# numz/ComfyUI-SeedVR2_VideoUpscaler

Hardware: NVIDIA H100
Metric: upscaled frames/sec SeedVR2-3B 720p->4K (higher is better)
Workload: dtype bf16

## Files before the change

comfyui-seedvr2_videoupscaler_b200/csrc/gemm.cu:

```cuda
#include <cuda.h>
#include <cuda_runtime.h>
#include <cuda_bf16.h>
#include <stdint.h>
#include <stdio.h>
#include <stdlib.h>

#include <type_traits>

#include "ptx.cuh"
#include "svr2_internal.h"

namespace svr2 {

constexpr int BLOCK_M = 128;
constexpr int BLOCK_K = 64;
constexpr int WGMMA_K = 16;

struct GemmParams {
  int M, N, K;
  int num_m_tiles, num_n_tiles, num_k_blocks;
  int band_h;
  int group_n;
  int a_mode;
  int tiles_w, tiles_h;
// ... 20 lines not shown
  const __nv_bfloat16* residual;
  void* out;
  float4* stat_partial;
  int stat_slots;
  const float* rowscale;
  float2* stat2;
  int ld_stat;
  const int* run_if;
  void* out2;
  void* out3;
  const int32_t* tok_dst;
  const int32_t* tok_rope;
  const float* rope_cos;
  const float* rope_sin;
  const float* qk_weight;
  float qk_eps;
  int qkv_inner;
};

enum : int {
  EPI_BIAS = 1,
  EPI_GATE = 2,
  EPI_RESIDUAL = 4,
  EPI_SWIGLU = 8,
  EPI_GELU = 16,
  EPI_F32 = 32,
  EPI_SHUFFLE = 64,
  EPI_SILU = 128,
  EPI_ROWSTAT = 256,
  EPI_PEXP = 512,
  EPI_ROWSCALE = 1024,
};

template <int BLOCK_N, bool EPI_WG>
struct SmemLayout {
  static constexpr int kABytes = BLOCK_M * BLOCK_K * 2;
  static constexpr int kBBytes = BLOCK_N * BLOCK_K * 2;
  static constexpr int kStageBytes = kABytes + kBBytes;
  static constexpr int kTileCols = BLOCK_N < 32 ? 32 : BLOCK_N;
  static constexpr int kStagingBytes = EPI_WG ? BLOCK_M * kTileCols * 2 : 8 * 4096;
  static constexpr int kBudget = 232448 - kStagingBytes - 256 - 1024;
  static constexpr int kStages = kBudget / kStageBytes > 8 ? 8 : kBudget / kStageBytes;
  static constexpr int kStagingOffset = kStages * kStageBytes;
  static constexpr int kBarOffset = kStagingOffset + kStagingBytes;
  static constexpr int kTotal = kBarOffset + 256 + 1024;
};

template <bool SWAP>
struct SlabLayout : SmemLayout<256, true> {
  using Base = SmemLayout<256, true>;
  static constexpr int kWBytes = (SWAP ? BLOCK_M : 256) * BLOCK_K * 2;
  static constexpr int kSBytes = (SWAP ? 32 * 10 : 16 * 10) * BLOCK_K * 2;
  static constexpr int kSStages = SWAP ? 2 : 3;
  static constexpr int kWStages = (Base::kBudget - kSStages * kSBytes) / kWBytes;
  static constexpr int kStages = kWStages + kSStages;
  static constexpr int kSlabOffset = kWStages * kWBytes;
  static constexpr int kStagingOffset = kSlabOffset + kSStages * kSBytes;
  static constexpr int kBarOffset = kStagingOffset + Base::kStagingBytes;
  static constexpr int kTotal = kBarOffset + 256 + 1024;
  static_assert(kWStages >= 3 && kSBytes % 1024 == 0 && kTotal <= 232448, "slab rings do not fit");
};

__device__ __forceinline__ void acc_ld32(const float* acc, uint32_t idx, uint32_t (&v)[32]) {
  const float4* s = reinterpret_cast<const float4*>(acc + idx);
#pragma unroll
  for (int i = 0; i < 8; ++i) {
    const float4 t = s[i];
    v[4 * i] = __float_as_uint(t.x); v[4 * i + 1] = __float_as_uint(t.y);
    v[4 * i + 2] = __float_as_uint(t.z); v[4 * i + 3] = __float_as_uint(t.w);
  }
}

__device__ __forceinline__ void stat_acc(float4& a, const uint4& d) {
// ... 22 lines not shown
  const int r = m_blk - band * full;
  const int rows_left = p.tiles_h - band * p.band_h;
  const int rows = rows_left < p.band_h ? rows_left : p.band_h;
  const int per = rows * p.tiles_w;
  t_o = r / per;
  const int rr = r - t_o * per;
  const int trow = rr / p.tiles_w;
  th = band * p.band_h + trow;
  tw = rr - trow * p.tiles_w;
}

__device__ __forceinline__ int conv_k_blocks(const GemmParams& p, int m_blk) {
  if (p.fold_t == 0) return p.num_k_blocks;
  int t_o, th, tw;
  conv_tile(p, m_blk, t_o, th, tw);
  return t_o < p.fold_t ? p.num_k_blocks - (p.taps_t - 1 - t_o) * p.taps_h * p.taps_w * p.cin_blocks : p.num_k_blocks;
}

__device__ __forceinline__ void tile_coords(int tile, int num_m, int num_n, int g, int& m, int& n) {
  const int per_group = g * num_m;
  const int ng = tile / per_group;
  const int r = tile - ng * per_group;
  const int n0 = ng * g;
  const int gsz = (num_n - n0) < g ? (num_n - n0) : g;
  m = r / gsz;
  n = n0 + (r - m * gsz);
}

enum : int { KIND_BF16 = 0, KIND_SWIGLU = 1, KIND_F32 = 2, KIND_ROWSTAT = 3, KIND_PEXP = 4,
             KIND_QKV21 = 5, KIND_QKV10 = 6,
             KIND_BF16_RS = 7,
             KIND_PEXP_STAT = 8 };

template <int KIND> constexpr bool kEpiWG = KIND == KIND_BF16;
constexpr int kNumThreads = 384;
constexpr int kEpiWarps = 2;

__device__ __forceinline__ int swap_tile_swz(int pix) { return ((pix & 1) << 2) | ((pix >> 1) & 3); }

struct RowDest {
  long long off;
  int valid;
  int dup;
};

template <int BLOCK_N>
__device__ __forceinline__ RowDest row_dest(const GemmParams& p, int epi, int m_blk, int n_blk, int row, int n_cols) {
  RowDest d;
  d.dup = 0;
  if (epi & EPI_SHUFFLE) {
    const int m = m_blk * BLOCK_M + row;
    d.valid = m < p.M;
    const int hw = p.shuf_H * p.shuf_W;
    const int f = m / hw, rr = m - f * hw, h = rr / p.shuf_W, w = rr - h * p.shuf_W;
    const int grp = (n_blk * BLOCK_N) / p.shuf_c;
    const int z = grp % p.shuf_z, y = (grp / p.shuf_z) & 1, x = grp / (p.shuf_z * 2);
    int t_out = f * p.shuf_z + z;
    if (p.shuf_drop) {
      if (f == 0 && z == 1) d.valid = 0;
      if (f > 0) t_out -= 1;
    }
    const int Wo = p.shuf_W * 2;
    const long long pix = (long long)(2 * h + x) * Wo + (2 * w + y);
    d.off = (long long)(t_out + p.out_t_pad) * p.out_frame_stride + pix * p.ldc + ((n_blk * BLOCK_N) % p.shuf_c);
    d.dup = (p.out_dup_head && t_out == 0 && d.valid) ? 1 : 0;
  } else if (p.a_mode == 0) {
    const int m = m_blk * BLOCK_M + row;
    d.valid = m < p.M;
    d.off = (long long)m * p.ldc + (long long)n_blk * n_cols;
  } else {
    int t_o, th, tw;
    conv_tile(p, m_blk, t_o, th, tw);
    const int rh = row / p.bw;
    const int h = th * p.bh + rh;
    const int w = tw * p.bw + (row - rh * p.bw);
    d.valid = (h < p.H_out) && (w < p.W_out);
    d.off = (long long)(t_o + p.out_t_pad) * p.out_frame_stride + ((long long)h * p.W_out + w) * p.ldc +
            (long long)n_blk * BLOCK_N;
    d.dup = (p.out_dup_head && t_o == 0 && d.valid) ? 1 : 0;
  }
  return d;
}

template <int BLOCK_N, int KIND, bool SWAP = false, int EPI_CT = -1, bool SLAB = false>
__global__ void __launch_bounds__(kNumThreads, 1)
gemm_wgmma_kernel(const __grid_constant__ CUtensorMap tmap_a, const __grid_constant__ CUtensorMap tmap_b,
                  const __grid_constant__ CUtensorMap tmap_a2, const GemmParams p) {
  if (p.run_if != nullptr && *p.run_if == 0) return;
  constexpr bool EPI_WG = kEpiWG<KIND>;
  static_assert(EPI_WG || (!SWAP && EPI_CT < 0), "swap-AB and compile-time epilogues are KIND_BF16 only");
  static_assert(!SLAB || (KIND == KIND_BF16 && BLOCK_N == 256), "the slab mainloop is KIND_BF16 with 256-column tiles");
  using S = SlabLayout<SWAP>;
  using L = std::conditional_t<SLAB, S, SmemLayout<BLOCK_N, EPI_WG>>;
  constexpr int kStages = L::kStages;
  constexpr int ACC_STRIDE = BLOCK_N < 32 ? 32 : BLOCK_N;
  constexpr int ACC_LD = ACC_STRIDE + 4;
  static_assert(EPI_WG || BLOCK_M * ACC_LD * 4 <= L::kStagingOffset, "the accumulator tile overlays the operand ring");
  extern __shared__ uint8_t smem_raw[];
  uint8_t* smem = reinterpret_cast<uint8_t*>((reinterpret_cast<uintptr_t>(smem_raw) + 1023) & ~uintptr_t(1023));
  uint64_t* full_bar = reinterpret_cast<uint64_t*>(smem + L::kBarOffset);
  uint64_t* empty_bar = full_bar + kStages;
  uint64_t* acc_free = empty_bar + kStages;
  uint64_t* tile_full = acc_free + 1;
  uint64_t* tile_empty = acc_free + 2;
  const float* acc_s = reinterpret_cast<const float*>(smem);
  uint8_t* tile_s = smem + L::kStagingOffset;

  const int warp = threadIdx.x >> 5;
  const int lane = threadIdx.x & 31;

  if (warp == 0 && lane == 0) {
    tma_prefetch_desc(&tmap_a);
    tma_prefetch_desc(&tmap_b);
    if (p.extra_blocks) tma_prefetch_desc(&tmap_a2);
  }
  if (warp == 1 && lane == 0) {
    for (int i = 0; i < kStages; ++i) {
      mbar_init(&full_bar[i], 1);
      mbar_init(&empty_bar[i], 2);
    }
    if constexpr (EPI_WG) {
      mbar_init(tile_full, 256);
      mbar_init(tile_empty, 32 * kEpiWarps);
    } else {
      mbar_init(acc_free, 256);
    }
    fence_barrier_init();
  }
  __syncthreads();

  const int num_n_tiles = p.num_n_tiles;
  const int num_m_tiles = p.num_m_tiles;
  const int num_tiles = num_m_tiles * num_n_tiles;
  const int tile0 = (int)blockIdx.x;
  const int tile_step = (int)gridDim.x;

  if (warp == 0 || warp == 3) {
    if constexpr (SLAB) {
      if (lane == 0) {
        const bool wgt = warp == 0;
        const int n_st = wgt ? S::kWStages : S::kSStages;
        const int bar0 = wgt ? 0 : S::kWStages;
        const int st_bytes = wgt ? S::kWBytes : S::kSBytes;
        uint8_t* const ring = smem + (wgt ? 0 : S::kSlabOffset);
        int stage = 0;
        uint32_t phase = 0;
        auto acquire = [&](uint32_t bytes, uint64_t*& fb) -> uint8_t* {
          mbar_wait(&empty_bar[bar0 + stage], phase ^ 1);
          fb = &full_bar[bar0 + stage];
          mbar_expect_tx(fb, bytes);
          uint8_t* s = ring + stage * st_bytes;
          if (++stage == n_st) { stage = 0; phase ^= 1; }
          return s;
        };
        const int bw = p.bw, bh = p.bh, taps_t = p.taps_t, cin_blocks = p.cin_blocks, cin = p.cin;
        const uint32_t slab_bytes = bw * (bh + 2) * BLOCK_K * 2, box_bytes = bw * bh * BLOCK_K * 2;
        for (int tile = tile0; tile < num_tiles; tile += tile_step) {
          int m_blk, n_blk, t_o, th, tw;
          tile_coords(tile, num_m_tiles, num_n_tiles, p.group_n, m_blk, n_blk);
          conv_tile(p, m_blk, t_o, th, tw);
          const int h0 = th * bh, w0 = tw * bw;
          int n0 = n_blk * (SWAP ? BLOCK_M : BLOCK_N);
          int taps = taps_t, kcol = 0;
          if (t_o < p.fold_t) {
            taps = t_o + 1;
            kcol = t_o == 0 ? 2 * 9 * cin : 0;
            n0 += p.fold_n;
          }
          uint64_t* fb;
          for (int kt_ = 0; kt_ < taps; ++kt_) {
// ... 2 lines not shown
              for (int cb = 0; cb < cin_blocks; ++cb) {
                if (wgt) {
                  for (int kh_ = 0; kh_ < 3; ++kh_) {
                    uint8_t* s = acquire(S::kWBytes, fb);
                    tma_load_2d(s, &tmap_b, fb, kcol + ((kt_ * 3 + kh_) * 3 + kw_) * cin + cb * BLOCK_K, n0);
                  }
                } else {
                  uint8_t* s = acquire(slab_bytes, fb);
                  tma_load_4d(s, &tmap_a, fb, cb * BLOCK_K, w0 + kw_ - p.pad_w, h0 - p.pad_h, t_in);
                }
              }
            }
          }
          kcol += taps * 9 * cin;
          for (int cb = 0; cb < p.extra_blocks; ++cb) {
            if (wgt) {
              uint8_t* s = acquire(S::kWBytes, fb);
              tma_load_2d(s, &tmap_b, fb, kcol + cb * BLOCK_K, n0);
            } else {
              uint8_t* s = acquire(box_bytes, fb);
              tma_load_4d(s, &tmap_a2, fb, cb * BLOCK_K, w0, h0, t_o);
            }
          }
        }
      }
    } else if (lane == 0) {
      int stage = 0;
      uint32_t phase = 0;
      uint32_t g = (warp == 0) ? 0u : 1u;
      uint32_t it = 0;
      const int a_mode = p.a_mode;
      const int nkb = p.num_k_blocks;
      auto acquire = [&](uint8_t*& sa, uint64_t*& fb) -> bool {
        const bool mine = (g++ & 1u) == 0u;
        if (mine) {
          mbar_wait(&empty_bar[stage], phase ^ 1);
          sa = smem + stage * L::kStageBytes;
          fb = &full_bar[stage];
          mbar_expect_tx(fb, L::kStageBytes);
        }
        return mine;
      };
      auto advance = [&]() {
        if (++stage == kStages) { stage = 0; phase ^= 1; }
      };
      auto tile_start = [&]() {
        if (!EPI_WG && it > 0) mbar_wait(acc_free, (it - 1) & 1u);
        ++it;
      };
      if (a_mode == 0) {
        for (int tile = tile0; tile < num_tiles; tile += tile_step) {
          int m_blk, n_blk;
          tile_coords(tile, num_m_tiles, num_n_tiles, p.group_n, m_blk, n_blk);
          tile_start();
          const int m0 = m_blk * BLOCK_M, n0 = n_blk * BLOCK_N;
          for (int kb = 0; kb < nkb; ++kb) {
            uint8_t* sa; uint64_t* fb;
            if (acquire(sa, fb)) {
              tma_load_2d(sa, &tmap_a, fb, kb * BLOCK_K, m0);
              tma_load_2d(sa + L::kABytes, &tmap_b, fb, kb * BLOCK_K, n0);
            }
            advance();
          }
        }
      } else {
        const int bw = p.bw, bh = p.bh, pad_h = p.pad_h, pad_w = p.pad_w, stride_t = p.stride_t;
        const int taps_t = p.taps_t, taps_h = p.taps_h, taps_w = p.taps_w, cin_blocks = p.cin_blocks, cin = p.cin;
// ... 147 lines not shown
#pragma unroll
          for (int i = 0; i < BLOCK_N / 2; i += 8) {
            const int pix = (i >> 3) * 16 + ((mj >> 1) << 3) + lr;
            stmatrix_x4_trans(tbase + pix * 256 + ((chunk ^ swap_tile_swz(pix)) << 4),
                              pack_bf16x2(d[i] + b0, d[i + 1] + b0), pack_bf16x2(d[i + 2] + b1, d[i + 3] + b1),
                              pack_bf16x2(d[i + 4] + b0, d[i + 5] + b0), pack_bf16x2(d[i + 6] + b1, d[i + 7] + b1));
          }
        } else {
          constexpr int ROW_B = L::kTileCols * 2;
          constexpr int SWZ = (L::kTileCols / 8 < 8 ? L::kTileCols / 8 : 8) - 1;
          const int row = r0 + ((mj & 1) << 3) + lr;
          const int cn0 = n_blk * BLOCK_N + 2 * (lane & 3);
#pragma unroll
          for (int i = 0; i < BLOCK_N / 2; i += 8) {
            float x[8];
#pragma unroll
            for (int e = 0; e < 8; ++e) x[e] = d[i + e];
            if (epi & EPI_BIAS) {
              const int cn = cn0 + (i >> 3) * 16;
              const uint32_t bl = cn < p.N ? __ldg(reinterpret_cast<const unsigned int*>(bias + cn)) : 0u;
              const uint32_t bh = cn + 8 < p.N ? __ldg(reinterpret_cast<const unsigned int*>(bias + cn + 8)) : 0u;
              x[0] += __uint_as_float(bl << 16); x[1] += __uint_as_float(bl & 0xffff0000u);
              x[2] += __uint_as_float(bl << 16); x[3] += __uint_as_float(bl & 0xffff0000u);
              x[4] += __uint_as_float(bh << 16); x[5] += __uint_as_float(bh & 0xffff0000u);
              x[6] += __uint_as_float(bh << 16); x[7] += __uint_as_float(bh & 0xffff0000u);
            }
            const int chunk = (i >> 3) * 2 + (mj >> 1);
            stmatrix_x4(tbase + row * ROW_B + ((chunk ^ (row & SWZ)) << 4), pack_bf16x2(x[0], x[1]),
                        pack_bf16x2(x[2], x[3]), pack_bf16x2(x[4], x[5]), pack_bf16x2(x[6], x[7]));
          }
        }
        mbar_arrive(tile_full);
      };
      for (int tile = tile0; tile < num_tiles; tile += tile_step, ++it) {
        int m_blk, n_blk;
        tile_coords(tile, num_m_tiles, num_n_tiles, p.group_n, m_blk, n_blk);
        auto store = [&](float (&d)[BLOCK_N / 2]) { store_tile(d, n_blk); };
        if constexpr (SLAB) mainloop_slab(conv_k_blocks(p, m_blk), store);
        else mainloop(conv_k_blocks(p, m_blk), store);
      }
    } else {
      auto acc_to_smem = [&](float (&d)[BLOCK_N / 2]) {
        named_bar_sync(1, 256);
        float* acc_w = reinterpret_cast<float*>(smem);
        const int r0 = wg * 64 + ((warp & 3) << 4) + (lane >> 2);
#pragma unroll
        for (int i = 0; i < BLOCK_N / 2; i += 4) {
          const int col = (i >> 2) * 8 + 2 * (lane & 3);
          *reinterpret_cast<float2*>(acc_w + r0 * ACC_LD + col) = make_float2(d[i], d[i + 1]);
          *reinterpret_cast<float2*>(acc_w + (r0 + 8) * ACC_LD + col) = make_float2(d[i + 2], d[i + 3]);
        }
        named_bar_sync(1, 256);
      };
      constexpr bool IS_BF16 = KIND == KIND_BF16_RS;
      constexpr bool IS_PEXP = KIND == KIND_PEXP || KIND == KIND_PEXP_STAT;
      constexpr int N_COLS = KIND == KIND_SWIGLU ? ACC_STRIDE / 2 : ACC_STRIDE;
      constexpr int COLS_W = N_COLS >= 64 ? N_COLS / 2 : N_COLS;
      constexpr int PH_COLS = KIND == KIND_F32 ? 32 : (COLS_W < 64 ? COLS_W : 64);
      constexpr int CPR = KIND == KIND_F32 ? PH_COLS / 4 : PH_COLS / 8;
      constexpr int ROWS_PER_IT = 32 / CPR;
      constexpr int N_IT = 32 / ROWS_PER_IT;
      constexpr int kBatch = N_IT < 4 ? N_IT : 4;
      const int q = warp & 3;
      const int half = (warp - 4) >> 2;
      const int row = q * 32 + lane;
      const bool active = (N_COLS >= 64) || (half == 0);
      const int col_lo = (N_COLS >= 64) ? half * COLS_W : 0;
      uint8_t* slab = smem + L::kStagingOffset + (warp - 4) * 4096;
      const int n_lim = KIND == KIND_SWIGLU ? p.N / 2 : p.N;
      const float* __restrict__ gate = p.gate;
      const __nv_bfloat16* __restrict__ resid = p.residual;
      for (int tile = tile0; tile < num_tiles; tile += tile_step) {
        int m_blk, n_blk;
        tile_coords(tile, num_m_tiles, num_n_tiles, p.group_n, m_blk, n_blk);
        if (it++ > 0) {
          fence_proxy_async_smem();
          mbar_arrive(acc_free);
        }
        mainloop(conv_k_blocks(p, m_blk), acc_to_smem);
        RowDest dst = row_dest<BLOCK_N>(p, epi, m_blk, n_blk, row, N_COLS);
        const int n_base = n_blk * (KIND == KIND_SWIGLU ? BLOCK_N / 2 : BLOCK_N);

        constexpr bool kWide = (IS_BF16 || IS_PEXP) && PH_COLS == 64;
        constexpr int N_PH = kWide ? COLS_W / 64 : 1;
        uint32_t bias_pk[N_PH];
        float2 gate2[N_PH];
        if constexpr (kWide && IS_BF16) {
#pragma unroll
          for (int ph = 0; ph < N_PH; ++ph) {
            const int cn = n_base + col_lo + ph * 64 + 2 * lane;
            const bool ok = cn < p.N;
            bias_pk[ph] = ((epi & EPI_BIAS) && ok) ? *reinterpret_cast<const uint32_t*>(bias + cn) : 0u;
            gate2[ph] = ((epi & EPI_GATE) && ok) ? *reinterpret_cast<const float2*>(gate + cn) : make_float2(0.f, 0.f);
          }
        }

        const uint32_t t_addr = row * ACC_LD;

        float row_lse = 0.f;
        float2 st_a = make_float2(0.f, 0.f), st_b = make_float2(0.f, 0.f);
        if constexpr (IS_PEXP) {
          const int m = m_blk * BLOCK_M + row;
          row_lse = (m < p.M) ? gate[m] : 0.f;
        }
        float row_scale = 1.f;
        if constexpr (KIND == KIND_BF16_RS) {
          const int m = m_blk * BLOCK_M + row;
          row_scale = (p.a_mode == 0 && m < p.M) ? p.rowscale[m] : 1.f;
        }
        if constexpr (KIND == KIND_QKV21 || KIND == KIND_QKV10) {
          static_assert(BLOCK_N == 256, "QKV epilogue needs 256-column tiles");
          constexpr int NF = KIND == KIND_QKV21 ? 21 : 10;
          const int tpw = p.qkv_inner / 256;
          const int which = n_blk / tpw;
          const int m = m_blk * BLOCK_M + row;
          const bool rvalid = (m < p.M);
          uint32_t pk[64];
#pragma unroll
          for (int c0 = 0; c0 < 128; c0 += 64) {
            uint32_t v0[32], v1[32];
            acc_ld32(acc_s, t_addr + col_lo + c0, v0);
            acc_ld32(acc_s, t_addr + col_lo + c0 + 32, v1);
#pragma unroll
            for (int i = 0; i < 16; ++i) {
              pk[c0 / 2 + i] = pack_bf16x2(__uint_as_float(v0[2 * i]), __uint_as_float(v0[2 * i + 1]));
              pk[c0 / 2 + 16 + i] = pack_bf16x2(__uint_as_float(v1[2 * i]), __uint_as_float(v1[2 * i + 1]));
            }
          }
          if (which < 2) {
            float ss = 0.f;
#pragma unroll
            for (int i = 0; i < 64; ++i) {
              const float lo = __uint_as_float(pk[i] << 16), hi = __uint_as_float(pk[i] & 0xffff0000u);
// ... 75 lines not shown
                float cm = -INFINITY;
#pragma unroll
                for (int j = 0; j < RS; ++j) {
                  const float t = (n0 + j < p.N) ? __uint_as_float(v[j]) * sc : -INFINITY;
                  v[j] = __float_as_uint(t);
                  cm = fmaxf(cm, t);
                }
                const float m_new = fmaxf(mx, cm);
                if (m_new > -INFINITY) {
                  float cs = 0.f;
#pragma unroll
                  for (int j = 0; j < RS; ++j) cs += exp2_approx(__uint_as_float(v[j]) - m_new);
                  sum = sum * exp2_approx(mx - m_new) + cs;
                  mx = m_new;
                }
              }
            }
          }
          const int m = m_blk * BLOCK_M + row;
          if (active && m < p.M) {
            const int slot = (N_COLS >= 64) ? n_blk * 2 + half : n_blk;
            reinterpret_cast<float2*>(p.out)[(long long)m * p.ldc + slot] = make_float2(mx, sum);
          }
        } else if (active) {
#pragma unroll 1
          for (int ph0 = col_lo; ph0 < col_lo + COLS_W; ph0 += PH_COLS) {
            if constexpr (kWide) {
              uint32_t v0[32], v1[32];
              acc_ld32(acc_s, t_addr + ph0, v0);
              acc_ld32(acc_s, t_addr + ph0 + 32, v1);
              const int phi = (ph0 - col_lo) / 64;
              uint32_t pk[32];
              const float sc = p.out_scale;
              constexpr bool want_stats = KIND == KIND_PEXP_STAT;
              const bool stats_full = n_base + ph0 + 64 <= p.N;
              const bool plain = !(epi & (EPI_GELU | EPI_SILU | EPI_GATE));
              auto elements = [&](auto ragged) {
#pragma unroll
              for (int i = 0; i < 32; ++i) {
                float a = __uint_as_float(i < 16 ? v0[2 * (i & 15)] : v1[2 * (i & 15)]);
                float b = __uint_as_float(i < 16 ? v0[2 * (i & 15) + 1] : v1[2 * (i & 15) + 1]);
                if constexpr (IS_PEXP) {
                  const bool kPoly = (KIND == KIND_PEXP_STAT) && ((i % 5 == 1) || (i % 5 == 3));
                  const float xa = fmaf(a, sc, -row_lse), xb = fmaf(b, sc, -row_lse);
                  const float ea = kPoly ? exp2_poly(xa) : exp2_approx(xa), eb = kPoly ? exp2_poly(xb) : exp2_approx(xb);
                  pk[i] = pack_bf16x2(ea, eb);
                  if constexpr (want_stats) {
                    if constexpr (decltype(ragged)::value) {
                      const int cn = n_base + ph0 + 2 * i;
                      if (cn < p.N) st_a.x += ea;
                      if (cn + 1 < p.N) st_a.y += eb;
                    } else {
                      if (i & 1) st_b = fadd2(st_b, make_float2(ea, eb));
                      else st_a = fadd2(st_a, make_float2(ea, eb));
                    }
                  }
                } else {
                  if constexpr (KIND == KIND_BF16_RS) {
                    a *= row_scale;
                    b *= row_scale;
                  }
                  if (epi & EPI_BIAS) {
                    const uint32_t bw_ = __shfl_sync(0xffffffffu, bias_pk[phi], i);
                    a += __uint_as_float(bw_ << 16);
                    b += __uint_as_float(bw_ & 0xffff0000u);
                  }
                  uint32_t r = pack_bf16x2(a, b);
                  if (!plain) {
                    if (epi & EPI_GELU) {
                      r = pack_bf16x2(gelu_tanh_fast(__uint_as_float(r << 16)), gelu_tanh_fast(__uint_as_float(r & 0xffff0000u)));
                    }
                    if (epi & EPI_SILU) {
                      r = pack_bf16x2(silu_fast(__uint_as_float(r << 16)), silu_fast(__uint_as_float(r & 0xffff0000u)));
                    }
                    if (epi & EPI_GATE) {
                      const float g0 = __shfl_sync(0xffffffffu, gate2[phi].x, i);
                      const float g1 = __shfl_sync(0xffffffffu, gate2[phi].y, i);
                      r = pack_bf16x2(__uint_as_float(r << 16) * g0, __uint_as_float(r & 0xffff0000u) * g1);
                    }
                  }
                  pk[i] = r;
                }
              }
              };
              if (want_stats && !stats_full) elements(std::true_type{});
              else elements(std::false_type{});
#pragma unroll
              for (int c = 0; c < 8; ++c)
                *reinterpret_cast<uint4*>(slab + lane * 128 + ((c ^ (lane & 7)) << 4)) =
                    make_uint4(pk[4 * c], pk[4 * c + 1], pk[4 * c + 2], pk[4 * c + 3]);
            } else {
#pragma unroll 1
            for (int c0 = ph0; c0 < ph0 + PH_COLS; c0 += 32) {
              uint32_t v[32];
              acc_ld32(acc_s, t_addr + c0, v);
              if constexpr (KIND == KIND_SWIGLU) {
                uint32_t u[32];
                acc_ld32(acc_s, t_addr + ACC_STRIDE / 2 + c0, u);
#pragma unroll
                for (int i = 0; i < 16; ++i) {
                  const uint32_t rg = pack_bf16x2(__uint_as_float(v[2 * i]), __uint_as_float(v[2 * i + 1]));
                  const uint32_t ru = pack_bf16x2(__uint_as_float(u[2 * i]), __uint_as_float(u[2 * i + 1]));
                  const uint32_t rs = pack_bf16x2(silu_fast(__uint_as_float(rg << 16)),
                                                  silu_fast(__uint_as_float(rg & 0xffff0000u)));
                  v[i] = pack_bf16x2(__uint_as_float(rs << 16) * __uint_as_float(ru << 16),
                                     __uint_as_float(rs & 0xffff0000u) * __uint_as_float(ru & 0xffff0000u));
                }
              } else if constexpr (KIND == KIND_F32) {
                const float sc = p.out_scale;
#pragma unroll
                for (int j = 0; j < 32; ++j) v[j] = __float_as_uint(__uint_as_float(v[j]) * sc);
              } else {
                static_assert(IS_PEXP, "the bf16 kinds take the wide path");
                const float sc = p.out_scale;
#pragma unroll
                for (int j = 0; j < 32; ++j)
                  v[j] = __float_as_uint(bf16_rne(exp2_approx(__uint_as_float(v[j]) * sc - row_lse)));
              }
              if constexpr (KIND == KIND_F32) {
// ... 29 lines not shown
            const bool col_ok = (n_base + col) < n_lim;
#pragma unroll 1
            for (int b0 = 0; b0 < N_IT; b0 += kBatch) {
              long long off[kBatch];
              int flags[kBatch];
              uint4 rv[kBatch];
#pragma unroll
              for (int i = 0; i < kBatch; ++i) {
                const int r = (b0 + i) * ROWS_PER_IT + rsub;
                off[i] = __shfl_sync(0xffffffffu, dst.off, r);
                const int f = __shfl_sync(0xffffffffu, dst.valid | (dst.dup << 1), r);
                flags[i] = col_ok ? f : 0;
                if constexpr (IS_BF16) {
                  if ((epi & EPI_RESIDUAL) && (flags[i] & 1)) rv[i] = *reinterpret_cast<const uint4*>(resid + off[i] + col);
                }
              }
#pragma unroll
              for (int i = 0; i < kBatch; ++i) {
                if (!(flags[i] & 1)) continue;
                const int r = (b0 + i) * ROWS_PER_IT + rsub;
                uint4 d = *reinterpret_cast<const uint4*>(slab + r * 128 + ((ch ^ (r & (CPR - 1))) << 4));
                if constexpr (KIND == KIND_F32) {
                  *reinterpret_cast<uint4*>(reinterpret_cast<float*>(p.out) + off[i] + col) = d;
                } else {
                  __nv_bfloat16* ob = reinterpret_cast<__nv_bfloat16*>(p.out);
                  if constexpr (IS_BF16) {
                    if (epi & EPI_RESIDUAL) d = add_bf16x8(d, rv[i]);
                  }
                  *reinterpret_cast<uint4*>(ob + off[i] + col) = d;
                }
              }
            }
            __syncwarp();
          }
          if constexpr (KIND == KIND_PEXP_STAT) {
            if (p.stat2) {
              const int m = m_blk * BLOCK_M + row;
              if (m < p.M) {
                const int slot = (N_COLS >= 64) ? n_blk * 2 + half : n_blk;
                p.stat2[(long long)m * p.ld_stat + slot] = make_float2(0.f, (st_a.x + st_b.x) + (st_a.y + st_b.y));
              }
            }
          }
        }
      }
    }
  } else {
    if constexpr (EPI_WG) {
      const int q0 = 2 * (warp - 1);
      const int epi = EPI_CT >= 0 ? EPI_CT : p.epi;
      const float* __restrict__ gate = p.gate;
      const __nv_bfloat16* __restrict__ resid = p.residual;
      __nv_bfloat16* ob = reinterpret_cast<__nv_bfloat16*>(p.out);
      uint32_t it = 0;
      for (int tile = tile0; tile < num_tiles; tile += tile_step, ++it) {
        int m_blk, n_blk;
        tile_coords(tile, num_m_tiles, num_n_tiles, p.group_n, m_blk, n_blk);
        mbar_wait(tile_full, it & 1u);
#pragma unroll 1
        for (int q = q0; q < q0 + 2; ++q) {
          const int row = q * 32 + lane;
          if constexpr (SWAP) {
            int t_o, th, tw;
            conv_tile(p, m_blk, t_o, th, tw);
            const int r = th * p.tiles_w + tw;
            const int h0 = th * p.bh, w0 = tw * p.bw;
            const long long fbase = (long long)(t_o + p.out_t_pad) * p.out_frame_stride + n_blk * BLOCK_M + q * 32;
            const bool dup_t = p.out_dup_head && t_o == 0;
            const int chn = lane & 3, psub = lane >> 2;
            const bool ch_ok = n_blk * BLOCK_M + q * 32 + chn * 8 < p.N;
#pragma unroll 1
            for (int half = 0; half < 2; ++half) {
              float4 st = make_float4(0.f, 0.f, 0.f, 0.f);
#pragma unroll 1
              for (int c0 = half * 128; c0 < half * 128 + 128; c0 += 32) {
                long long off[4];
                int flags[4];
                uint4 rv[4];
#pragma unroll
                for (int i = 0; i < 4; ++i) {
                  const int pj = c0 + i * 8 + psub;
// ... 150 lines not shown
    estr[i] = 1;
    if (i > 0) gstr[i - 1] = strides_bytes[i - 1];
  }
  CUresult r = enc(map, CU_TENSOR_MAP_DATA_TYPE_BFLOAT16, rank, const_cast<void*>(base), gdim, gstr, bdim, estr,
                   CU_TENSOR_MAP_INTERLEAVE_NONE, CU_TENSOR_MAP_SWIZZLE_128B, CU_TENSOR_MAP_L2_PROMOTION_L2_256B,
                   CU_TENSOR_MAP_FLOAT_OOB_FILL_NONE);
  if (r != CUDA_SUCCESS) {
    char msg[256];
    snprintf(msg, sizeof msg, "cuTensorMapEncodeTiled failed (%d) rank=%d dims=%llu,%llu,%llu box=%u,%u,%u", (int)r,
             rank, (unsigned long long)dims[0], (unsigned long long)(rank > 1 ? dims[1] : 0),
             (unsigned long long)(rank > 2 ? dims[2] : 0), box[0], rank > 1 ? box[1] : 0, rank > 2 ? box[2] : 0);
    return set_error(SVR2_ERR_CUDA, msg);
  }
  return SVR2_OK;
}

constexpr int kMaxDevices = 64;
int current_device() {
  int dev = 0;
  cudaGetDevice(&dev);
  return (dev >= 0 && dev < kMaxDevices) ? dev : 0;
}
static int g_num_sms[kMaxDevices] = {};
int num_sms() {
  const int dev = current_device();
  if (!g_num_sms[dev]) cudaDeviceGetAttribute(&g_num_sms[dev], cudaDevAttrMultiProcessorCount, dev);
  return g_num_sms[dev];
}

template <int BLOCK_N, int KIND, bool SWAP = false, int EPI_CT = -1, bool SLAB = false>
static int launch_gemm(const CUtensorMap& ta, const CUtensorMap& tb, const GemmParams& p_in, cudaStream_t stream,
                       const CUtensorMap* ta2_opt = nullptr) {
  const CUtensorMap& ta2 = ta2_opt ? *ta2_opt : ta;
  using L = std::conditional_t<SLAB, SlabLayout<SWAP>, SmemLayout<BLOCK_N, kEpiWG<KIND>>>;
  auto kern = gemm_wgmma_kernel<BLOCK_N, KIND, SWAP, EPI_CT, SLAB>;
  GemmParams p = p_in;
  {
    const long long b_tile_bytes = (long long)(SWAP ? BLOCK_M : BLOCK_N) * p.num_k_blocks * BLOCK_K * 2;
    long long g = (16LL << 20) / (b_tile_bytes > 0 ? b_tile_bytes : 1);
    if (g < 1) g = 1;
    if (g > p.num_n_tiles) g = p.num_n_tiles;
    p.group_n = (int)g;
  }
  static bool configured[kMaxDevices] = {};
  const int dev = current_device();
  if (!configured[dev]) {
    cudaError_t e = cudaFuncSetAttribute(kern, cudaFuncAttributeMaxDynamicSharedMemorySize, L::kTotal);
    if (e != cudaSuccess) return set_error(SVR2_ERR_CUDA, cudaGetErrorString(e));
    configured[dev] = true;
  }
  int tiles = p.num_m_tiles * p.num_n_tiles;
  int grid = tiles < num_sms() ? tiles : num_sms();
  if (grid <= 0) return SVR2_OK;
  kern<<<grid, kNumThreads, L::kTotal, stream>>>(ta, tb, ta2, p);
  cudaError_t e = cudaGetLastError();
  if (e != cudaSuccess) return set_error(SVR2_ERR_CUDA, cudaGetErrorString(e));
  return SVR2_OK;
}

static int dispatch_gemm(int block_n, const CUtensorMap& ta, const CUtensorMap& tb, const GemmParams& p,
                         cudaStream_t s, const CUtensorMap* ta2 = nullptr) {
  if (ta2) {
    switch (block_n) {
      case 256: return launch_gemm<256, KIND_BF16>(ta, tb, p, s, ta2);
      case 128: return launch_gemm<128, KIND_BF16>(ta, tb, p, s, ta2);
    }
    return set_error(SVR2_ERR_ARG, "fused shortcut: Cout must be >= 128");
  }
  if (p.epi & EPI_ROWSCALE) {
    if (block_n == 256) return launch_gemm<256, KIND_BF16_RS>(ta, tb, p, s);
    if (block_n == 128) return launch_gemm<128, KIND_BF16_RS>(ta, tb, p, s);
    return set_error(SVR2_ERR_ARG, "EPI_ROWSCALE needs >= 128-column tiles");
  }
  if ((p.epi & EPI_PEXP) && p.stat2) {
    if (block_n != 256) return set_error(SVR2_ERR_ARG, "EPI_PEXP statistics need 256-column tiles");
    return launch_gemm<256, KIND_PEXP_STAT>(ta, tb, p, s);
  }
  if (p.epi & EPI_SWIGLU) {
    if (block_n == 256) return launch_gemm<256, KIND_SWIGLU>(ta, tb, p, s);
    return set_error(SVR2_ERR_ARG, "SwiGLU epilogue needs BLOCK_N = 256");
  }
  if (p.epi & EPI_ROWSTAT) {
    if (block_n == 256) return launch_gemm<256, KIND_ROWSTAT>(ta, tb, p, s);
    if (block_n == 128) return launch_gemm<128, KIND_ROWSTAT>(ta, tb, p, s);
    if (block_n == 64) return launch_gemm<64, KIND_ROWSTAT>(ta, tb, p, s);
    return launch_gemm<32, KIND_ROWSTAT>(ta, tb, p, s);
  }
  if (p.epi & EPI_PEXP) {
    if (block_n == 256) return launch_gemm<256, KIND_PEXP>(ta, tb, p, s);
    if (block_n == 128) return launch_gemm<128, KIND_PEXP>(ta, tb, p, s);
    if (block_n == 64) return launch_gemm<64, KIND_PEXP>(ta, tb, p, s);
    return launch_gemm<32, KIND_PEXP>(ta, tb, p, s);
  }
  if (p.epi & EPI_F32) {
    switch (block_n) {
      case 256: return launch_gemm<256, KIND_F32>(ta, tb, p, s);
      case 128: return launch_gemm<128, KIND_F32>(ta, tb, p, s);
      case 64: return launch_gemm<64, KIND_F32>(ta, tb, p, s);
      case 32: return launch_gemm<32, KIND_F32>(ta, tb, p, s);
      case 16: return launch_gemm<16, KIND_F32>(ta, tb, p, s);
    }
  }
  if (block_n == 256) {
    switch (p.epi) {
      case EPI_SHUFFLE | EPI_BIAS: return launch_gemm<256, KIND_BF16, false, EPI_SHUFFLE | EPI_BIAS>(ta, tb, p, s);
      case EPI_BIAS | EPI_GATE | EPI_RESIDUAL: return launch_gemm<256, KIND_BF16, false, EPI_BIAS | EPI_GATE | EPI_RESIDUAL>(ta, tb, p, s);
      case EPI_GATE | EPI_RESIDUAL: return launch_gemm<256, KIND_BF16, false, EPI_GATE | EPI_RESIDUAL>(ta, tb, p, s);
      case EPI_BIAS: return launch_gemm<256, KIND_BF16, false, EPI_BIAS>(ta, tb, p, s);
      case 0: return launch_gemm<256, KIND_BF16, false, 0>(ta, tb, p, s);
// ... 346 lines not shown
```

Before: 1.559.

## Overlap PEXP_STAT epilogue via fp32 smem handoff to three epilogue warps

For the probability-exp-with-stats GEMM kind, the math warpgroups now write fp32 accumulators into a double-buffered, swizzled shared-memory tile and signal per-half barriers. Three dedicated epilogue warps (including the former second producer warp) compute exp2, row sums and the bf16 stores, while the math warps continue with the next tile's mainloop. The aim is to take the expensive exponent epilogue off the WGMMA critical path. In exchange, the larger staging buffer reduces the number of pipeline stages, and a single producer warp now issues all loads.

```diff
diff --git a/comfyui-seedvr2_videoupscaler_b200/csrc/gemm.cu b/comfyui-seedvr2_videoupscaler_b200/csrc/gemm.cu
--- a/comfyui-seedvr2_videoupscaler_b200/csrc/gemm.cu
+++ b/comfyui-seedvr2_videoupscaler_b200/csrc/gemm.cu
@@ -76,13 +76,15 @@
   EPI_ROWSCALE = 1024,
 };
 
-template <int BLOCK_N, bool EPI_WG>
+constexpr int kF32EpiWarps = 3;
+
+template <int BLOCK_N, bool EPI_WG, bool F32_TILE = false>
 struct SmemLayout {
   static constexpr int kABytes = BLOCK_M * BLOCK_K * 2;
   static constexpr int kBBytes = BLOCK_N * BLOCK_K * 2;
   static constexpr int kStageBytes = kABytes + kBBytes;
   static constexpr int kTileCols = BLOCK_N < 32 ? 32 : BLOCK_N;
-  static constexpr int kStagingBytes = EPI_WG ? BLOCK_M * kTileCols * 2 : 8 * 4096;
+  static constexpr int kStagingBytes = F32_TILE ? 2 * 64 * BLOCK_N * 4 : EPI_WG ? BLOCK_M * kTileCols * 2 : 8 * 4096;
   static constexpr int kBudget = 232448 - kStagingBytes - 256 - 1024;
   static constexpr int kStages = kBudget / kStageBytes > 8 ? 8 : kBudget / kStageBytes;
   static constexpr int kStagingOffset = kStages * kStageBytes;
@@ -171,9 +173,23 @@
              KIND_BF16_RS = 7,
              KIND_PEXP_STAT = 8 };
 
-template <int KIND> constexpr bool kEpiWG = KIND == KIND_BF16;
+template <int KIND> constexpr bool kF32Tile = KIND == KIND_PEXP_STAT;
+template <int KIND> constexpr bool kEpiWG = KIND == KIND_BF16 || kF32Tile<KIND>;
 constexpr int kNumThreads = 384;
 constexpr int kEpiWarps = 2;
+
+template <int BLOCK_N, int KIND>
+using GemmLayout = SmemLayout<BLOCK_N, kEpiWG<KIND>, kF32Tile<KIND>>;
+
+__device__ __forceinline__ void f32_tile_ld32(const float* row_p, int c, int swz, uint32_t (&v)[32]) {
+  const float4* s = reinterpret_cast<const float4*>(row_p);
+#pragma unroll
+  for (int i = 0; i < 8; ++i) {
+    const float4 t = s[(c * 8 + i) ^ swz];
+    v[4 * i] = __float_as_uint(t.x); v[4 * i + 1] = __float_as_uint(t.y);
+    v[4 * i + 2] = __float_as_uint(t.z); v[4 * i + 3] = __float_as_uint(t.w);
+  }
+}
 
 __device__ __forceinline__ int swap_tile_swz(int pix) { return ((pix & 1) << 2) | ((pix >> 1) & 3); }
 
@@ -227,10 +243,12 @@
                   const __grid_constant__ CUtensorMap tmap_a2, const GemmParams p) {
   if (p.run_if != nullptr && *p.run_if == 0) return;
   constexpr bool EPI_WG = kEpiWG<KIND>;
-  static_assert(EPI_WG || (!SWAP && EPI_CT < 0), "swap-AB and compile-time epilogues are KIND_BF16 only");
+  constexpr bool F32_TILE = kF32Tile<KIND>;
+  static_assert(KIND == KIND_BF16 || (!SWAP && EPI_CT < 0), "swap-AB and compile-time epilogues are KIND_BF16 only");
   static_assert(!SLAB || (KIND == KIND_BF16 && BLOCK_N == 256), "the slab mainloop is KIND_BF16 with 256-column tiles");
+  static_assert(!F32_TILE || BLOCK_N == 256, "the fp32 handoff is laid out for 256-column tiles");
   using S = SlabLayout<SWAP>;
-  using L = std::conditional_t<SLAB, S, SmemLayout<BLOCK_N, EPI_WG>>;
+  using L = std::conditional_t<SLAB, S, GemmLayout<BLOCK_N, KIND>>;
   constexpr int kStages = L::kStages;
   constexpr int ACC_STRIDE = BLOCK_N < 32 ? 32 : BLOCK_N;
   constexpr int ACC_LD = ACC_STRIDE + 4;
@@ -241,7 +259,7 @@
   uint64_t* empty_bar = full_bar + kStages;
   uint64_t* acc_free = empty_bar + kStages;
   uint64_t* tile_full = acc_free + 1;
-  uint64_t* tile_empty = acc_free + 2;
+  uint64_t* tile_empty = acc_free + 3;
   const float* acc_s = reinterpret_cast<const float*>(smem);
   uint8_t* tile_s = smem + L::kStagingOffset;
 
@@ -258,7 +276,12 @@
       mbar_init(&full_bar[i], 1);
       mbar_init(&empty_bar[i], 2);
     }
-    if constexpr (EPI_WG) {
+    if constexpr (F32_TILE) {
+      for (int h = 0; h < 2; ++h) {
+        mbar_init(&tile_full[h], 128);
+        mbar_init(&tile_empty[h], 32 * kF32EpiWarps);
+      }
+    } else if constexpr (EPI_WG) {
       mbar_init(tile_full, 256);
       mbar_init(tile_empty, 32 * kEpiWarps);
     } else {
@@ -274,7 +297,7 @@
   const int tile0 = (int)blockIdx.x;
   const int tile_step = (int)gridDim.x;
 
-  if (warp == 0 || warp == 3) {
+  if (warp == 0 || (warp == 3 && !F32_TILE)) {
     if constexpr (SLAB) {
       if (lane == 0) {
         const bool wgt = warp == 0;
@@ -343,7 +366,7 @@
       const int a_mode = p.a_mode;
       const int nkb = p.num_k_blocks;
       auto acquire = [&](uint8_t*& sa, uint64_t*& fb) -> bool {
-        const bool mine = (g++ & 1u) == 0u;
+        const bool mine = F32_TILE || (g++ & 1u) == 0u;
         if (mine) {
           mbar_wait(&empty_bar[stage], phase ^ 1);
           sa = smem + stage * L::kStageBytes;
@@ -557,10 +580,26 @@
         }
         mbar_arrive(tile_full);
       };
+      auto store_f32 = [&](float (&d)[BLOCK_N / 2]) {
+        if (it > 0) mbar_wait(&tile_empty[wg], (it - 1) & 1u);
+        float* buf = reinterpret_cast<float*>(tile_s) + wg * 64 * BLOCK_N;
+        const int r = ((warp & 3) << 4) + (lane >> 2);
+        const int swz = r & 7;
+#pragma unroll
+        for (int i = 0; i < BLOCK_N / 2; i += 4) {
+          const int e = ((((i >> 2) * 2 + ((lane >> 1) & 1)) ^ swz) << 2) + 2 * (lane & 1);
+          *reinterpret_cast<float2*>(buf + r * BLOCK_N + e) = make_float2(d[i], d[i + 1]);
+          *reinterpret_cast<float2*>(buf + (r + 8) * BLOCK_N + e) = make_float2(d[i + 2], d[i + 3]);
+        }
+        mbar_arrive(&tile_full[wg]);
+      };
       for (int tile = tile0; tile < num_tiles; tile += tile_step, ++it) {
         int m_blk, n_blk;
         tile_coords(tile, num_m_tiles, num_n_tiles, p.group_n, m_blk, n_blk);
-        auto store = [&](float (&d)[BLOCK_N / 2]) { store_tile(d, n_blk); };
+        auto store = [&](float (&d)[BLOCK_N / 2]) {
+          if constexpr (F32_TILE) store_f32(d);
+          else store_tile(d, n_blk);
+        };
         if constexpr (SLAB) mainloop_slab(conv_k_blocks(p, m_blk), store);
         else mainloop(conv_k_blocks(p, m_blk), store);
       }
@@ -578,7 +617,7 @@
         named_bar_sync(1, 256);
       };
       constexpr bool IS_BF16 = KIND == KIND_BF16_RS;
-      constexpr bool IS_PEXP = KIND == KIND_PEXP || KIND == KIND_PEXP_STAT;
+      constexpr bool IS_PEXP = KIND == KIND_PEXP;
       constexpr int N_COLS = KIND == KIND_SWIGLU ? ACC_STRIDE / 2 : ACC_STRIDE;
       constexpr int COLS_W = N_COLS >= 64 ? N_COLS / 2 : N_COLS;
       constexpr int PH_COLS = KIND == KIND_F32 ? 32 : (COLS_W < 64 ? COLS_W : 64);
@@ -623,7 +662,6 @@
         const uint32_t t_addr = row * ACC_LD;
 
         float row_lse = 0.f;
-        float2 st_a = make_float2(0.f, 0.f), st_b = make_float2(0.f, 0.f);
         if constexpr (IS_PEXP) {
           const int m = m_blk * BLOCK_M + row;
           row_lse = (m < p.M) ? gate[m] : 0.f;
@@ -765,29 +803,13 @@
               const int phi = (ph0 - col_lo) / 64;
               uint32_t pk[32];
               const float sc = p.out_scale;
-              constexpr bool want_stats = KIND == KIND_PEXP_STAT;
-              const bool stats_full = n_base + ph0 + 64 <= p.N;
               const bool plain = !(epi & (EPI_GELU | EPI_SILU | EPI_GATE));
-              auto elements = [&](auto ragged) {
 #pragma unroll
               for (int i = 0; i < 32; ++i) {
                 float a = __uint_as_float(i < 16 ? v0[2 * (i & 15)] : v1[2 * (i & 15)]);
                 float b = __uint_as_float(i < 16 ? v0[2 * (i & 15) + 1] : v1[2 * (i & 15) + 1]);
                 if constexpr (IS_PEXP) {
-                  const bool kPoly = (KIND == KIND_PEXP_STAT) && ((i % 5 == 1) || (i % 5 == 3));
-                  const float xa = fmaf(a, sc, -row_lse), xb = fmaf(b, sc, -row_lse);
-                  const float ea = kPoly ? exp2_poly(xa) : exp2_approx(xa), eb = kPoly ? exp2_poly(xb) : exp2_approx(xb);
-                  pk[i] = pack_bf16x2(ea, eb);
-                  if constexpr (want_stats) {
-                    if constexpr (decltype(ragged)::value) {
-                      const int cn = n_base + ph0 + 2 * i;
-                      if (cn < p.N) st_a.x += ea;
-                      if (cn + 1 < p.N) st_a.y += eb;
-                    } else {
-                      if (i & 1) st_b = fadd2(st_b, make_float2(ea, eb));
-                      else st_a = fadd2(st_a, make_float2(ea, eb));
-                    }
-                  }
+                  pk[i] = pack_bf16x2(exp2_approx(fmaf(a, sc, -row_lse)), exp2_approx(fmaf(b, sc, -row_lse)));
                 } else {
                   if constexpr (KIND == KIND_BF16_RS) {
                     a *= row_scale;
@@ -815,9 +837,6 @@
                   pk[i] = r;
                 }
               }
-              };
-              if (want_stats && !stats_full) elements(std::true_type{});
-              else elements(std::false_type{});
 #pragma unroll
               for (int c = 0; c < 8; ++c)
                 *reinterpret_cast<uint4*>(slab + lane * 128 + ((c ^ (lane & 7)) << 4)) =
@@ -914,20 +933,103 @@
             }
             __syncwarp();
           }
-          if constexpr (KIND == KIND_PEXP_STAT) {
-            if (p.stat2) {
-              const int m = m_blk * BLOCK_M + row;
-              if (m < p.M) {
-                const int slot = (N_COLS >= 64) ? n_blk * 2 + half : n_blk;
-                p.stat2[(long long)m * p.ld_stat + slot] = make_float2(0.f, (st_a.x + st_b.x) + (st_a.y + st_b.y));
-              }
-            }
-          }
         }
       }
     }
   } else {
-    if constexpr (EPI_WG) {
+    if constexpr (F32_TILE) {
+      const float* __restrict__ lse = p.gate;
+      __nv_bfloat16* ob = reinterpret_cast<__nv_bfloat16*>(p.out);
+      const float sc = p.out_scale;
+      const int e = warp - 1;
+      const int swz = lane & 7;
+      uint32_t it = 0;
+      for (int tile = tile0; tile < num_tiles; tile += tile_step, ++it) {
+        int m_blk, n_blk;
+        tile_coords(tile, num_m_tiles, num_n_tiles, p.group_n, m_blk, n_blk);
+        const int n_base = n_blk * BLOCK_N;
+#pragma unroll 1
+        for (int h = 0; h < 2; ++h) {
+          float lse_q[2];
+#pragma unroll
+          for (int qh = 0; qh < 2; ++qh) {
+            const int m = m_blk * BLOCK_M + (2 * h + qh) * 32 + lane;
+            lse_q[qh] = m < p.M ? lse[m] : 0.f;
+          }
+          float* half_buf = reinterpret_cast<float*>(tile_s) + h * 64 * BLOCK_N;
+          mbar_wait(&tile_full[h], it & 1u);
+#pragma unroll 1
+          for (int j = ((e - 4 * h) % kF32EpiWarps + kF32EpiWarps) % kF32EpiWarps; j < 4; j += kF32EpiWarps) {
+            const int qh = j >> 1, half = j & 1;
+            const int row = (2 * h + qh) * 32 + lane;
+            const int m = m_blk * BLOCK_M + row;
+            const float row_lse = qh ? lse_q[1] : lse_q[0];
+            const RowDest dst = row_dest<BLOCK_N>(p, p.epi, m_blk, n_blk, row, BLOCK_N);
+            float* quad = half_buf + qh * 32 * BLOCK_N;
+            const float* row_p = quad + lane * BLOCK_N;
+            float2 st_a = make_float2(0.f, 0.f), st_b = make_float2(0.f, 0.f);
+#pragma unroll 1
+            for (int ph0 = half * 128; ph0 < half * 128 + 128; ph0 += 64) {
+              uint32_t v0[32], v1[32], pk[32];
+              f32_tile_ld32(row_p, ph0 / 32, swz, v0);
+              f32_tile_ld32(row_p, ph0 / 32 + 1, swz, v1);
+              auto elements = [&](auto ragged) {
+#pragma unroll
+                for (int i = 0; i < 32; ++i) {
+                  const float a = __uint_as_float(i < 16 ? v0[2 * (i & 15)] : v1[2 * (i & 15)]);
+                  const float b = __uint_as_float(i < 16 ? v0[2 * (i & 15) + 1] : v1[2 * (i & 15) + 1]);
+                  const bool kPoly = (i % 5 == 1) || (i % 5 == 3);
+                  const float xa = fmaf(a, sc, -row_lse), xb = fmaf(b, sc, -row_lse);
+                  const float ea = kPoly ? exp2_poly(xa) : exp2_approx(xa), eb = kPoly ? exp2_poly(xb) : exp2_approx(xb);
+                  pk[i] = pack_bf16x2(ea, eb);
+                  if constexpr (decltype(ragged)::value) {
+                    const int cn = n_base + ph0 + 2 * i;
+                    if (cn < p.N) st_a.x += ea;
+                    if (cn + 1 < p.N) st_a.y += eb;
+                  } else {
+                    if (i & 1) st_b = fadd2(st_b, make_float2(ea, eb));
+                    else st_a = fadd2(st_a, make_float2(ea, eb));
+                  }
+                }
+              };
+              if (n_base + ph0 + 64 <= p.N) elements(std::false_type{});
+              else elements(std::true_type{});
+              uint8_t* slab = reinterpret_cast<uint8_t*>(quad + ph0);
+#pragma unroll
+              for (int c = 0; c < 8; ++c)
+                *reinterpret_cast<uint4*>(slab + lane * (BLOCK_N * 4) + ((c ^ swz) << 4)) =
+                    make_uint4(pk[4 * c], pk[4 * c + 1], pk[4 * c + 2], pk[4 * c + 3]);
+              __syncwarp();
+              const int ch = lane & 7, rsub = lane >> 3;
+              const int col = ph0 + ch * 8;
+              const bool col_ok = n_base + col < p.N;
+#pragma unroll 1
+              for (int b0 = 0; b0 < 8; b0 += 4) {
+                long long off[4];
+                int ok[4];
+#pragma unroll
+                for (int i = 0; i < 4; ++i) {
+                  const int r = (b0 + i) * 4 + rsub;
+                  off[i] = __shfl_sync(0xffffffffu, dst.off, r);
+                  ok[i] = __shfl_sync(0xffffffffu, dst.valid, r) && col_ok;
+                }
+#pragma unroll
+                for (int i = 0; i < 4; ++i) {
+                  if (!ok[i]) continue;
+                  const int r = (b0 + i) * 4 + rsub;
+                  *reinterpret_cast<uint4*>(ob + off[i] + col) =
+                      *reinterpret_cast<const uint4*>(slab + r * (BLOCK_N * 4) + ((ch ^ (r & 7)) << 4));
+                }
+              }
+              __syncwarp();
+            }
+            if (p.stat2 && m < p.M)
+              p.stat2[(long long)m * p.ld_stat + n_blk * 2 + half] = make_float2(0.f, (st_a.x + st_b.x) + (st_a.y + st_b.y));
+          }
+          mbar_arrive(&tile_empty[h]);
+        }
+      }
+    } else if constexpr (EPI_WG) {
       const int q0 = 2 * (warp - 1);
       const int epi = EPI_CT >= 0 ? EPI_CT : p.epi;
       const float* __restrict__ gate = p.gate;
@@ -1144,7 +1246,7 @@
 static int launch_gemm(const CUtensorMap& ta, const CUtensorMap& tb, const GemmParams& p_in, cudaStream_t stream,
                        const CUtensorMap* ta2_opt = nullptr) {
   const CUtensorMap& ta2 = ta2_opt ? *ta2_opt : ta;
-  using L = std::conditional_t<SLAB, SlabLayout<SWAP>, SmemLayout<BLOCK_N, kEpiWG<KIND>>>;
+  using L = std::conditional_t<SLAB, SlabLayout<SWAP>, GemmLayout<BLOCK_N, KIND>>;
   auto kern = gemm_wgmma_kernel<BLOCK_N, KIND, SWAP, EPI_CT, SLAB>;
   GemmParams p = p_in;
   {
```

Result: no change. 1.564 (median of 6 runs) (+0.3%).

## Compute softmax probabilities and row sums directly in MMA warpgroup registers

Applied to the files above, without the earlier changes.

The PEXP_STAT GEMM kind now uses the epilogue-warpgroup path. The math warpgroups exponentiate accumulators in registers, write bf16 probabilities to shared memory with stmatrix, and reduce the row sums with warp shuffles. This replaces the round trip through the accumulator staging buffer and the separate epilogue-warp exponent pass. It moves exp work (mixed poly/approx exp2) onto the MMA warps, which can lengthen the mainloop's critical path, and it changes which columns use the polynomial exp.

```diff
diff --git a/comfyui-seedvr2_videoupscaler_b200/csrc/gemm.cu b/comfyui-seedvr2_videoupscaler_b200/csrc/gemm.cu
--- a/comfyui-seedvr2_videoupscaler_b200/csrc/gemm.cu
+++ b/comfyui-seedvr2_videoupscaler_b200/csrc/gemm.cu
@@ -171,7 +171,7 @@
              KIND_BF16_RS = 7,
              KIND_PEXP_STAT = 8 };
 
-template <int KIND> constexpr bool kEpiWG = KIND == KIND_BF16;
+template <int KIND> constexpr bool kEpiWG = KIND == KIND_BF16 || KIND == KIND_PEXP_STAT;
 constexpr int kNumThreads = 384;
 constexpr int kEpiWarps = 2;
 
@@ -557,12 +557,54 @@
         }
         mbar_arrive(tile_full);
       };
+      const int rq = r0 + (lane >> 2);
+      auto pexp_tile = [&](float (&d)[BLOCK_N / 2], int m, int n_blk, float mh0, float mh1) {
+        static_assert(KIND != KIND_PEXP_STAT || (BLOCK_N == 256 && !SWAP), "the single-pass probabilities use 256-column tiles");
+        const float sc = p.out_scale;
+        const int n_left = p.N - (n_blk * BLOCK_N + 2 * (lane & 3));
+        const int row = r0 + ((mj & 1) << 3) + lr;
+        const uint32_t abase = tbase + row * (BLOCK_N * 2);
+        float st[4] = {};
+        if (it > 0) mbar_wait(tile_empty, (it - 1) & 1u);
+#pragma unroll
+        for (int k = 0; k < BLOCK_N / 16; ++k) {
+          uint32_t pk[4];
+#pragma unroll
+          for (int e = 0; e < 4; ++e) {
+            const int j = 4 * k + e;
+            const bool poly = j >= 8 && j % 3 == 1;
+            const float mh = (j & 1) ? mh1 : mh0;
+            const float xa = fmaf(d[2 * j], sc, -mh), xb = fmaf(d[2 * j + 1], sc, -mh);
+            const float ea = poly ? exp2_poly(xa) : exp2_approx(xa), eb = poly ? exp2_poly(xb) : exp2_approx(xb);
+            pk[e] = pack_bf16x2(ea, eb);
+            if (8 * (j >> 1) < n_left) st[(j & 1) * 2 + (j >> 5)] += ea + eb;
+          }
+          stmatrix_x4(abase + ((k >> 2) << 7) + (((2 * (k & 3) + (mj >> 1)) ^ (row & 7)) << 4), pk[0], pk[1], pk[2],
+                      pk[3]);
+        }
+        mbar_arrive(tile_full);
+#pragma unroll
+        for (int k = 0; k < 4; ++k) {
+          st[k] += __shfl_xor_sync(0xffffffffu, st[k], 1);
+          st[k] += __shfl_xor_sync(0xffffffffu, st[k], 2);
+        }
+        const int q = lane & 3;
+        const int mq = m + ((q >> 1) << 3);
+        const float v = q == 0 ? st[0] : q == 1 ? st[1] : q == 2 ? st[2] : st[3];
+        if (mq < p.M) p.stat2[(long long)mq * p.ld_stat + 2 * n_blk + (q & 1)] = make_float2(0.f, v);
+      };
       for (int tile = tile0; tile < num_tiles; tile += tile_step, ++it) {
         int m_blk, n_blk;
         tile_coords(tile, num_m_tiles, num_n_tiles, p.group_n, m_blk, n_blk);
-        auto store = [&](float (&d)[BLOCK_N / 2]) { store_tile(d, n_blk); };
-        if constexpr (SLAB) mainloop_slab(conv_k_blocks(p, m_blk), store);
-        else mainloop(conv_k_blocks(p, m_blk), store);
+        if constexpr (KIND == KIND_PEXP_STAT) {
+          const int m = m_blk * BLOCK_M + rq;
+          const float mh0 = m < p.M ? p.gate[m] : 0.f, mh1 = m + 8 < p.M ? p.gate[m + 8] : 0.f;
+          mainloop(p.num_k_blocks, [&](float (&d)[BLOCK_N / 2]) { pexp_tile(d, m, n_blk, mh0, mh1); });
+        } else {
+          auto store = [&](float (&d)[BLOCK_N / 2]) { store_tile(d, n_blk); };
+          if constexpr (SLAB) mainloop_slab(conv_k_blocks(p, m_blk), store);
+          else mainloop(conv_k_blocks(p, m_blk), store);
+        }
       }
     } else {
       auto acc_to_smem = [&](float (&d)[BLOCK_N / 2]) {
@@ -578,7 +620,7 @@
         named_bar_sync(1, 256);
       };
       constexpr bool IS_BF16 = KIND == KIND_BF16_RS;
-      constexpr bool IS_PEXP = KIND == KIND_PEXP || KIND == KIND_PEXP_STAT;
+      constexpr bool IS_PEXP = KIND == KIND_PEXP;
       constexpr int N_COLS = KIND == KIND_SWIGLU ? ACC_STRIDE / 2 : ACC_STRIDE;
       constexpr int COLS_W = N_COLS >= 64 ? N_COLS / 2 : N_COLS;
       constexpr int PH_COLS = KIND == KIND_F32 ? 32 : (COLS_W < 64 ? COLS_W : 64);
@@ -623,7 +665,6 @@
         const uint32_t t_addr = row * ACC_LD;
 
         float row_lse = 0.f;
-        float2 st_a = make_float2(0.f, 0.f), st_b = make_float2(0.f, 0.f);
         if constexpr (IS_PEXP) {
           const int m = m_blk * BLOCK_M + row;
           row_lse = (m < p.M) ? gate[m] : 0.f;
@@ -765,29 +806,13 @@
               const int phi = (ph0 - col_lo) / 64;
               uint32_t pk[32];
               const float sc = p.out_scale;
-              constexpr bool want_stats = KIND == KIND_PEXP_STAT;
-              const bool stats_full = n_base + ph0 + 64 <= p.N;
               const bool plain = !(epi & (EPI_GELU | EPI_SILU | EPI_GATE));
-              auto elements = [&](auto ragged) {
 #pragma unroll
               for (int i = 0; i < 32; ++i) {
                 float a = __uint_as_float(i < 16 ? v0[2 * (i & 15)] : v1[2 * (i & 15)]);
                 float b = __uint_as_float(i < 16 ? v0[2 * (i & 15) + 1] : v1[2 * (i & 15) + 1]);
                 if constexpr (IS_PEXP) {
-                  const bool kPoly = (KIND == KIND_PEXP_STAT) && ((i % 5 == 1) || (i % 5 == 3));
-                  const float xa = fmaf(a, sc, -row_lse), xb = fmaf(b, sc, -row_lse);
-                  const float ea = kPoly ? exp2_poly(xa) : exp2_approx(xa), eb = kPoly ? exp2_poly(xb) : exp2_approx(xb);
-                  pk[i] = pack_bf16x2(ea, eb);
-                  if constexpr (want_stats) {
-                    if constexpr (decltype(ragged)::value) {
-                      const int cn = n_base + ph0 + 2 * i;
-                      if (cn < p.N) st_a.x += ea;
-                      if (cn + 1 < p.N) st_a.y += eb;
-                    } else {
-                      if (i & 1) st_b = fadd2(st_b, make_float2(ea, eb));
-                      else st_a = fadd2(st_a, make_float2(ea, eb));
-                    }
-                  }
+                  pk[i] = pack_bf16x2(exp2_approx(fmaf(a, sc, -row_lse)), exp2_approx(fmaf(b, sc, -row_lse)));
                 } else {
                   if constexpr (KIND == KIND_BF16_RS) {
                     a *= row_scale;
@@ -815,9 +840,6 @@
                   pk[i] = r;
                 }
               }
-              };
-              if (want_stats && !stats_full) elements(std::true_type{});
-              else elements(std::false_type{});
 #pragma unroll
               for (int c = 0; c < 8; ++c)
                 *reinterpret_cast<uint4*>(slab + lane * 128 + ((c ^ (lane & 7)) << 4)) =
@@ -913,15 +935,6 @@
               }
             }
             __syncwarp();
-          }
-          if constexpr (KIND == KIND_PEXP_STAT) {
-            if (p.stat2) {
-              const int m = m_blk * BLOCK_M + row;
-              if (m < p.M) {
-                const int slot = (N_COLS >= 64) ? n_blk * 2 + half : n_blk;
-                p.stat2[(long long)m * p.ld_stat + slot] = make_float2(0.f, (st_a.x + st_b.x) + (st_a.y + st_b.y));
-              }
-            }
           }
         }
       }
@@ -1186,7 +1199,7 @@
   }
   if ((p.epi & EPI_PEXP) && p.stat2) {
     if (block_n != 256) return set_error(SVR2_ERR_ARG, "EPI_PEXP statistics need 256-column tiles");
-    return launch_gemm<256, KIND_PEXP_STAT>(ta, tb, p, s);
+    return launch_gemm<256, KIND_PEXP_STAT, false, EPI_PEXP>(ta, tb, p, s);
   }
   if (p.epi & EPI_SWIGLU) {
     if (block_n == 256) return launch_gemm<256, KIND_SWIGLU>(ta, tb, p, s);
```

Result: no change. 1.569 before, 1.584 after, median of 6 (+0.9%).
